# jaeyoungchoilab/Topsicle

Measured on AMD Instinct MI355X. Metric: bases_scanned_per_sec, higher is better.
Workload: dtype u8

## Files before the change

### __graft_entry__.py

```python
import os
import shutil
import subprocess
import sys

ROOT = os.path.dirname(os.path.abspath(__file__))
CSRC = os.path.join(ROOT, "topsicle_amd", "csrc")
LIB = os.path.join(ROOT, "topsicle_amd", "libtopsicle_hip.so")


def _newer(target, deps):
    return os.path.exists(target) and all(os.path.getmtime(target) >= os.path.getmtime(d) for d in deps)


HIP_FLAGS = ["--offload-arch=gfx950", "-O3", "-fno-vectorize", "-std=c++17", "-fPIC", "-Wall", "-Wno-unused-variable"]
KGROUPS = 18


def _build_hip_split(out, extra=()):
    hipcc = shutil.which("hipcc") or "/opt/rocm/bin/hipcc"
    flags = os.environ.get("TPS_HIPCC_EXTRA", "").split() + HIP_FLAGS + list(extra)
    bdir = os.path.join(CSRC, "_build", os.path.splitext(os.path.basename(out))[0])
    os.makedirs(bdir, exist_ok=True)
    jobs = []
    for g in range(KGROUPS):
# ... 24 lines not shown
    out = os.path.join(ROOT, "topsicle_amd", "libtopsicle_io.so")
    if not force and _newer(out, [src, os.path.join(CSRC, "tps_pack.h"), os.path.join(CSRC, "tps_gzpar.h"), os.path.join(ROOT, "include", "topsicle_hip.h")]):
        return out
    subprocess.check_call(["g++", "-O2", "-std=c++17", "-shared", "-fPIC", "-Wall", "-o", out, src, "-lz", "-lpthread"])
    return out


def build_oracle():
    mk = os.path.join(ROOT, "oracle", "Makefile")
    if os.path.exists(mk):
        subprocess.check_call(["make", "-s", "-C", os.path.join(ROOT, "oracle")])


def build_emulation():
    sys.path.insert(0, os.path.join(ROOT, "tests"))
    sys.path.insert(0, ROOT)
    import emu_adapter_driver
    import emu_anchor_driver
    import emu_binseg_driver
    import emu_clear_driver
    import emu_driver
    import emu_ends_driver
    import emu_follow_wide_driver
    import emu_motif_driver
    import emu_place_driver
    import emu_refine_driver
    import emu_tract_driver
    import emu_variant_driver
    import emu_wide_driver
    emu_driver.build()
    emu_binseg_driver.build()
    emu_wide_driver.build()
    emu_wide_driver.build_main()
    emu_follow_wide_driver.build()
    emu_motif_driver.build()
    emu_motif_driver.build_main()
    emu_variant_driver.build()
    emu_variant_driver.build_main()
    emu_tract_driver.build()
    emu_tract_driver.build_main()
    emu_ends_driver.build()
    emu_ends_driver.build_main()
    emu_anchor_driver.build()
    emu_anchor_driver.build_main()
    emu_place_driver.build()
    emu_place_driver.build_main()
    emu_adapter_driver.build()
    emu_adapter_driver.build_main()
    emu_refine_driver.build()
    emu_refine_driver.build_main()
    emu_clear_driver.build_main()
    import test_layout
    test_layout.build_main()

# ... 111 lines not shown
```

### topsicle_amd/csrc/topsicle_hip.hip

```cpp
#include <hip/hip_runtime.h>
#include <hip/hip_ext.h>

#include <sys/uio.h>
#include <unistd.h>

#include <algorithm>
#include <cerrno>
#include <cstdarg>
#include <cstdio>
#include <cstdlib>
#include <cstring>
#include <deque>
#include <initializer_list>
#include <map>
#include <mutex>
#include <set>
#include <string>
#include <vector>

#include "tps_device.h"
#include "tps_motif.h"
#include "tps_variant.h"
#include "tps_tract.h"
#include "tps_ends.h"
// ... 371 lines not shown
    size_t table_rr = 0;
    DevBuf follow_picks, follow_hist;
    DevBuf motif_hits, motif_counts;
    DevBuf variant_in, variant_counts, variant_prof;
    std::vector<unsigned long long> h_variant_prof;
    DevBuf tract_table, tract_out;
    DevBuf ends_in, ends_out;
    DevBuf links_t, links_out;
    DevBuf window_out;
    DevBuf offsets_in, offsets_out;
    DevBuf place_in, place_idx, place_out;
    DevBuf adapter_in, adapter_out;
    DevBuf refine_in, refine_out;
    DevBuf ascii, ascii_off;
    DevBuf nib, nib_src;
    std::set<void*> pinned;
    std::vector<tps_read_desc> h_desc;
    tps::PatInfo pat{};
    bool have_pat = false;
    Slot slots[TPS_MAX_SLOTS + 1];
    std::vector<EventPair> ev_pool;
    size_t ev_used = 0;
    size_t ev_base = 0;
    tps::PlanKnobs knobs{};
    int want_stamps = 0;
    int no_events = 0;
    int no_inline_rows = 0;
    int no_stride = 0;
    int file_order = 0;
    int poison = 0;
    int event_stride = 1;
    uint64_t launch_seq = 0;
    size_t lds_set_refine = 0;
    size_t lds_set_generic = 0;
    size_t lds_set_fused[KF_COUNT][KSLIDE_MAX - KSLIDE_MIN + 1] = {};
    uint32_t* h_flag = nullptr;
    hipEvent_t share_ev = nullptr;
    void* raw_stage[2] = {nullptr, nullptr};
    hipEvent_t raw_ev[2] = {nullptr, nullptr};
};

namespace {

int bind(tps_ctx* c) {
    if (!c) return fail(TPS_E_ARG, "null context");
    HIP_TRY(hipSetDevice(c->device));
    return TPS_OK;
// ... 1585 lines not shown
    double tot = 0.0;
    for (size_t i = c->ev_base; i < c->ev_used; ++i) {
        float ms = 0.f;
        HIP_TRY(hipEventElapsedTime(&ms, c->ev_pool[i].a, c->ev_pool[i].b));
        tot += ms;
    }
    const size_t cnt = c->ev_used - c->ev_base;
    if (n_launches) *n_launches = (int32_t)cnt;
    if (total_ms) *total_ms = tot;
    if (mean_ms) *mean_ms = cnt ? tot / (double)cnt : 0.0;
    return TPS_OK;
}

int tps_ctx_debug_option(tps_ctx* c, const char* key, int64_t value) {
    if (!c || !key) return fail(TPS_E_ARG, "null argument");
    const std::string k(key);
    if (k == "event_stride") c->event_stride = (int)std::max<int64_t>(1, value);
    else if (k == "no_events") c->no_events = value != 0;
    else if (k == "force_generic") c->knobs.force_generic = value != 0;
    else if (k == "spans_per_tile") c->knobs.spans_per_tile = (int)std::max<int64_t>(0, value);
    else if (k == "force_pair") c->knobs.force_pair = value != 0;
    else if (k == "so_order") c->knobs.so_order = (int)value;
    else if (k == "wpg") c->knobs.wpg = (int)value;
    else if (k == "stamps") c->want_stamps = value != 0;
    else if (k == "file_order") c->file_order = value != 0;
    else if (k == "no_stride") c->no_stride = value != 0;
    else if (k == "no_inline_rows") c->no_inline_rows = value != 0;
    else if (k == "poison") {
        if (value < 0 || value > 255) return fail(TPS_E_ARG, "poison must be 0 (off) or a fill byte 1..255");
        c->poison = (int)value;
    }
    else return fail(TPS_E_ARG, "unknown debug option '%s' (event_stride, no_events, force_generic, spans_per_tile, force_pair, so_order, wpg, stamps, file_order, no_stride, no_inline_rows, poison)", key);
    drop_plans(c);
    return TPS_OK;
}

int tps_debug_stamps_get(tps_ctx* c, int32_t slot, uint64_t* out, int64_t n) {
    Slot* sl;
    int rc;
    if ((rc = need_scanned(c, slot, &sl))) return rc;
    if (!sl->stamps.p || n != sl->n) return fail(TPS_E_STATE, "no stamps recorded");
    HIP_TRY(hipMemcpy(out, sl->stamps.p, (size_t)n * 16 * 8, hipMemcpyDeviceToHost));
    return TPS_OK;
}

int tps_kernel_time_reset(tps_ctx* c) {
    int rc;
    if ((rc = bind(c))) return rc;
    HIP_TRY(hipStreamSynchronize(c->stream));
    c->ev_base = c->ev_used;
    c->launch_seq = 0;
    return TPS_OK;
}

}
// ... 1 lines not shown
```

### topsicle_amd/csrc/tps_device.h

```cpp
#pragma once
#include <stdint.h>
#include "../../include/topsicle_hip.h"
#include "tps_wave.h"
#include "tps_check.h"

namespace tps {

constexpr int WPG = 4;
constexpr int WPG_MAX = 8;
constexpr uint32_t FLAG_CONFLICT = 0x80000000u;
constexpr uint32_t FLAG16 = 0x8000u;
constexpr int HIST_COPIES = 8;
constexpr int WIN_U = 4;
constexpr int COOP_MAX = 24;

typedef unsigned __int128 u128;

constexpr int cgcd(int a, int b) { return b == 0 ? a : cgcd(b, a % b); }
constexpr int clog2(int x) { return x <= 1 ? 0 : 1 + clog2(x / 2); }

struct PatInfo {
    int32_t P, k;
    uint32_t kmask;
    uint32_t all_mask;
// ... 38 lines not shown
    int32_t blk_log2;
    int32_t rec_rs;
    int32_t tot_dw;
    int32_t blk_dw;
    int32_t lc_cap;
    uint32_t jump_magic;
    int32_t q, r, lw;
    int32_t lc_global;
    int32_t lc_stride;
    uint16_t* lc_scratch;
    int32_t pair_n;
    int32_t tw;
    int32_t tile_full;
    int32_t wpg;
    int32_t pp_d;
    int32_t so_fast;
    int32_t val_on;
    int32_t seq_alias;
    int32_t lut_fields;
    int32_t lut16;
    int32_t xt_alias;
    int32_t xt_own;
    int32_t pair16;
};

struct BinsegArgs {
    const int32_t* sums;
    const int64_t* win_off;
    int32_t* bkp;
    double* gain;
    int64_t n_reads;
    int32_t n_patterns, jump, min_size;
    uint8_t* tie;
};

constexpr int MISC_DW = 20;
constexpr int XS_DW = 64 + NT + 4 * NT + NT + 16 * 5 + 8;
constexpr int HIST_STRIDE = 33;
constexpr int HIST_DW = 2 * HIST_COPIES * HIST_STRIDE;
struct Lds {
    uint32_t* lut;
    uint32_t* lut2;
    int lshift;
    uint32_t* seq2;
    uint16_t* val;
    uint32_t* blk;
    uint32_t* G;
    uint32_t* Gp;
    uint16_t* C0;
    uint16_t* C1;
    uint32_t* XPC;
    uint32_t* XF;
    uint32_t* XT;
    uint32_t* Tot;
    uint32_t* row;
    uint32_t* misc;
};
constexpr int XLANES = NT + 16;
TPS_HD int64_t xchg_dw(const ScanArgs& a) {
    return 9ll * NT + (a.xt_alias == 2 ? 0ll : 2ll) * XLANES;
}
TPS_HD int64_t lut_dw(const ScanArgs& a) { return a.lut16 ? ((((int64_t)a.lut_n + 1) / 2 + 3) & ~3ll) : (((int64_t)a.lut_n + 3) & ~3ll); }
TPS_HD int64_t blk_region_dw(const ScanArgs& a) {
    int64_t need = a.variant ? xchg_dw(a) : 2ll * a.nblk_cap + 2ll * ((a.nblk_cap + 1) / 2);
    if (need < XS_DW) need = XS_DW;
    if (need < HIST_DW) need = HIST_DW;
    return (need + 3) & ~3ll;
}
TPS_HD int64_t val_dw(const ScanArgs& a) { return a.val_on ? ((a.seq_dw + 4 + 3) / 4) * 2 : 0; }
TPS_HD int64_t row_dw(const ScanArgs& a) {
    const int64_t fused = a.variant ? ((int64_t)NT << a.blk_log2) + NT : 0;
    return fused > WIN_U * NT ? fused : WIN_U * NT;
}
TPS_DEV Lds carve(uint32_t* base, uint32_t* lut, const ScanArgs& a) {
    Lds l;
    l.lut2 = lut - a.pair_n;
    uint32_t* p = base;
    l.blk = p;  p += a.blk_dw;
    l.lut = lut;
    l.lshift = a.variant ? 16 : 0;
    l.seq2 = p; p += a.seq_dw;
    l.val = (uint16_t*)p;  p += val_dw(a);
    l.Tot = p;  p += a.tot_dw;
    l.row = p;  p += row_dw(a);
    l.misc = p;
    l.G = l.blk;
    l.Gp = l.G + a.nblk_cap;
    l.C0 = (uint16_t*)(l.Gp + a.nblk_cap);
    l.C1 = l.C0 + ((a.nblk_cap + 1) / 2) * 2;
    l.XPC = l.blk;
    l.XF = l.XPC + 9 * NT;
    l.XT = l.XF + XLANES;
    return l;
}
TPS_HD int64_t lds_dwords(const ScanArgs& a) {
    return (int64_t)a.blk_dw + (a.seq_alias ? 0 : a.seq_dw) + val_dw(a) + a.tot_dw + row_dw(a) + MISC_DW +
           ((a.xt_alias && a.xt_own) ? (a.xt_alias == 2 ? 2 : 1) * XLANES : 0);
}
TPS_HD int64_t wg_lds_dwords(const ScanArgs& a) { return a.pair_n + lut_dw(a) + (int64_t)(a.wpg > 0 ? a.wpg : WPG) * ((lds_dwords(a) + 3) & ~3ll); }
constexpr int M_BEST = 0;
constexpr int M_CMASK = 2;
constexpr int M_INVALID = 4;
constexpr int M_SCAN = 10;
constexpr int M_MAXSC = 6;
constexpr int M_BESTB = 8;
constexpr int M_NTIE = 9;
constexpr int X_Q = 0;
constexpr int X_BS = 64;
// ... 758 lines not shown
    return t;
}

template <int S>
struct Geo {
    static constexpr int B = 8;
    static constexpr int LOG2B = 3;
    static constexpr int C = 8;
    static constexpr int LOG2C = 3;
    static constexpr int POS = B * S;
    static constexpr int WDW = (POS + 13 + 15) / 16;
};
constexpr int SEQ_LEAD = 4;
template <int S, bool FULL>
struct TileGeo {
    static constexpr int LANES = FULL ? NT : NT - 1;
    static constexpr int BASES = LANES * Geo<S>::POS + 13 + 15;
    static constexpr int NQ = (63 + BASES + 63) / 64;
    static constexpr int PF = (NQ + NT - 1) / NT;
    static constexpr int SEQ_TILE = SEQ_LEAD + 4 * NQ + 4;
    static constexpr int SEQ = SEQ_TILE < 144 ? 144 : SEQ_TILE;
};
constexpr bool tile_full_default(int s) { return s >= 1; }

template <int S, bool FULL>
TPS_DEV Lds carve_fused(uint32_t* base, uint32_t* lut, const ScanArgs& a) {
    constexpr int BLK = 9 * NT, ROW = NT * Geo<S>::B + NT, SEQ = TileGeo<S, FULL>::SEQ;
    const int VAL = a.val_on ? ((SEQ + 4 + 3) / 4) * 2 : 0;
    static_assert(BLK % 4 == 0 && ROW % 4 == 0 && MISC_DW % 4 == 0 && SEQ % 4 == 0, "seq2 must be 16-byte aligned");
    static_assert(BLK + ROW - SEQ >= HIST_DW && BLK + ROW - SEQ >= 4 * NT, "step 1 counts in front of the aliased bases");
    Lds l;
    l.lut2 = lut - a.pair_n;
    l.lut = lut;
    l.lshift = (a.lut16 && !a.lut_fields && !a.pair16) ? LUT_M16 : (a.lut_fields && a.lut16) ? LUT_F16 : a.lut_fields ? LUT_FIELDS : 16;
    l.blk = base;
    l.XPC = base;
    l.G = l.Gp = base; l.C0 = l.C1 = (uint16_t*)base;
    l.row = base + BLK;
    l.misc = l.row + ROW;
    l.Tot = l.misc + MISC_DW;
    uint32_t* p = l.Tot + 4;
    if (a.seq_alias) {
        l.seq2 = base + (BLK + ROW - SEQ);
    } else {
        l.seq2 = p;
        p += SEQ;
    }
    l.val = (uint16_t*)p;
    p += VAL;
    l.XF = p;
    l.XT = l.XF + XLANES;
    return l;
}

TPS_DEV uint32_t pack_hi_lo(uint32_t hi_src, uint32_t lo_src) { return perm(hi_src, lo_src, 0x07060100u); }

template <int S, bool SO, bool INV, int RPT, bool RAW>
TPS_DEV void tile_fused_s(const ScanArgs& a, const TileConst& tc, const Lds& l, int delta, int w0, int tile, int nw_tile,
                          int64_t out_base, uint64_t& s_total, int64_t r) {
    constexpr bool RZ = RPT == 0;
    typedef Geo<S> g_;
    constexpr int WDW = g_::WDW, B = g_::B, LOG2B = g_::LOG2B, POS = g_::POS;
    constexpr int RS = NT + NT / B;
    const PatInfo& pat = a.pat;
    const int rp = RPT >= 0 ? RPT : tc.r, q = tc.q;
// ... 686 lines not shown
            }
        } else {
            TPS_EMU_COUNT(6);
        }
    }
    const Lane<uint32_t> lexc = wave_excl_sum(ltot);
    bool lane_cands = false;
    if constexpr (CD == 0 && !M16) lane_cands = tc.jump >= 4u;
    const uint32_t c_lo = div_jump((uint32_t)w0 + tc.jump - 1u, tc.jump_magic);
    uint32_t c_hi = div_jump((uint32_t)(w0 + nw_tile) + tc.jump - 1u, tc.jump_magic);
    if (c_hi > tc.lc_cap) c_hi = tc.lc_cap;
    TPS_PHASE {
        const int lane = tid;
        const uint32_t* const sw = TPS_AT(sw_);
        if constexpr (SWP) g_store_sw8p(tc.sw16 + w0, lane, nw_tile, TPS_AT(swp_));
        else g_store_sw8(tc.sw16 + w0, lane, nw_tile, sw);
        uint32_t* pr = l.row + lane * (B + 1);
        uint32_t run = 0;
        TPS_UNROLL
        for (int j = 0; j < B; ++j) { pr[j] = run; run += sw[j]; }
        xt_at(lane) = TPS_AT(lexc);
        if (lane_cands) {
            if (tid == 0) TPS_EMU_COUNT(7);
            auto own_candidates = [&](auto bigj_) {
                const uint32_t carry = (uint32_t)s_total + TPS_AT(lexc);
                const uint32_t wa = (uint32_t)w0 + (uint32_t)(lane * B);
                const uint32_t c = mulhi32(wa + tc.jump - 1u, tc.jump_magic);
                const uint32_t f = c * tc.jump - wa, f2 = f + tc.jump;
                uint32_t i1 = c, r1 = f;
                if constexpr (decltype(bigj_)::value != 0) {
                    i1 = f < (uint32_t)B ? c : c_hi;
                    r1 = f < (uint32_t)B ? f : (uint32_t)(B - 1);
                }
                const uint32_t i2 = (f2 < (uint32_t)B ? c : c_hi) + 1u;
                const uint32_t r2 = f2 < (uint32_t)B ? f2 : (uint32_t)(B - 1);
                const uint32_t v1 = pr[r1], v2 = pr[r2];
                g32_store_clamped(tc.lc_g, c_hi, i1, carry + v1);
                g32_store_clamped(tc.lc_g, c_hi, i2, carry + v2);
            };
            if (tc.jump > (uint32_t)B) own_candidates(IntC<1>());
            else own_candidates(IntC<0>());
        }
    }
    TPS_SYNC();
    if (w0 == 0) TPS_STAMP(12);
    TPS_ISA_MARK(MK + 4);
    const uint32_t gsum = uniform(l.row[nw_tile + (nw_tile >> LOG2B)] + xt_at(nw_tile >> LOG2B));
    {
        const uint32_t jump = tc.jump;
        const int passes = (c_hi > c_lo && !lane_cands) ? (int)((c_hi - c_lo + NT - 1) / NT) : 0;
        TPS_ISA_MARK(MK + 6);
        TPS_PHASE {
            const uint32_t carry = (uint32_t)s_total;
            if (tid == 0) { l.misc[M_INVALID] = 0; l.misc[M_NTIE] = 0; }
            uint32_t c = c_lo + (uint32_t)tid;
            uint32_t w = c * jump - (uint32_t)w0;
            TPS_NOVEC
            for (int t = 0; t < passes; ++t) {
                if (c < c_hi) {
                    const uint32_t pre = l.row[w + (w >> LOG2B)] + xt_at((int)(w >> LOG2B));
                    g32_store(tc.lc_g, c, carry + pre);
                }
                c += NT;
                w += NT * jump;
// ... 643 lines not shown
        const int best_b = TPS_AT(best_b_);
        double m;
        __builtin_memcpy(&m, &misc[M_MAXSC], 8);
        const double thr = m * (1.0 - 1e-14);
        uint32_t near = (best >= thr && best >= 0.0 ? 1u : 0u) + (second >= thr && second >= 0.0 ? 1u : 0u);
        if (near) lds_add(&misc[M_NTIE], near);
        if (best == m && best_b >= 0) lds_max_i32((int32_t*)&misc[M_BESTB], best_b);
    }
    TPS_SYNC();
    tie = misc[M_NTIE] > 1u;
    if (tie) {
        Cand ex = binseg_exact_wg(S, n, jump, min_size, xs);
        bkp = ex.b;
        gain = ex.b < 0 ? 0.0 : gain_from((int64_t)ex.d, ex.den, n, n_patterns);
    } else {
        bkp = (int32_t)misc[M_BESTB];
        double m;
        __builtin_memcpy(&m, &misc[M_MAXSC], 8);
        gain = bkp < 0 ? 0.0 : m / (double)n / ((double)n_patterns * (double)n_patterns);
        TPS_SYNC();
    }
}

template <typename ST>
TPS_DEV void binseg_from_lc(const ScanArgs& a, const Lds& l, uint64_t lc_g, const ST* S_global, int n, uint64_t tot, int jump,
                            int min_size, int n_patterns, uint32_t* misc, uint32_t* xs, int& bkp, double& gain, bool& tie) {
    const int ncand = (n - 1) / jump;
    Lane<double> best_(-1.0);
    Lane<int> best_b_(-1);
    Lane<bool> amb_(false);
    Lane<uint64_t> bits_(0);
    const int c_min = (min_size + jump - 1) / jump > 1 ? (min_size + jump - 1) / jump : 1;
    const int c_max = (n - min_size) / jump < ncand ? (n - min_size) / jump : ncand;
    const bool exact53 = (double)n * 4294967296.0 < 9007199254740992.0 && (double)tot * (double)n < 9007199254740992.0;
    const double nf = (double)n, totf = (double)tot;
    const bool int_d = (double)tot * (double)n < 2147483648.0 && tot < (1ull << 24);
    constexpr int LCV = 16;
    const bool prefilter = exact53 && c_max - c_min < LCV * NT;
    int nslot = c_max >= c_min ? (c_max - c_min + NT) / NT : 0;
    TPS_PIN_S(nslot);
    Lane<float> p_s1_(-1.0f), p_s2_(-1.0f);
    Lane<uint32_t> p_lc_(0);
    Lane<int> p_c_(-1);
    float thr32 = -1.0f;
    bool crowded = false;
    TPS_ISA_REGION(5);
    if (prefilter) {
        auto prefilter_phase = [&](auto intd_) {
        TPS_PHASE {
            constexpr bool INTD = decltype(intd_)::value != 0;
            float &p_s1 = TPS_AT(p_s1_), &p_s2 = TPS_AT(p_s2_);
            uint32_t& p_lc = TPS_AT(p_lc_);
            p_s1 = -1.0f; p_s2 = -1.0f; p_lc = 0;
            int p_j = -1;
            const int c0 = c_min + tid;
            const uint32_t off0 = 4u * (uint32_t)c0;
            const float nf32 = (float)n, bstep = (float)(NT * jump);
            float bf = (float)(c0 * jump);
            const uint32_t ntb_step = 0u - (uint32_t)tot * (uint32_t)(NT * jump);
            uint32_t ntb = 0u - (uint32_t)tot * (uint32_t)(c0 * jump);
            auto slot = [&](int j, uint32_t lc, auto last_) {
                float d32;
                if constexpr (INTD) {
                    d32 = (float)(int32_t)(mul24((uint32_t)n, lc) + ntb);
                    ntb += ntb_step;
                } else {
                    d32 = (float)__builtin_fma(-totf, (double)bf, nf * (double)lc);
                }
                const float den32 = bf * (nf32 - bf);
                bf += bstep;
                float s_ = d32 * d32 * rcp_f32(den32);
                if constexpr (decltype(last_)::value != 0) s_ = tid <= c_max - c_min - j * NT ? s_ : -1.0f;
                const bool gt = s_ > p_s1;
                p_s2 = med3_f32(p_s1, p_s2, s_);
                p_lc = gt ? lc : p_lc;
                p_j = gt ? j : p_j;
                p_s1 = gt ? s_ : p_s1;
            };
            auto group = [&](int g, auto checked_) {
                constexpr bool CHECKED = decltype(checked_)::value != 0;
                uint32_t lcv[4];
                TPS_UNROLL
                for (int i = 0; i < 4; ++i) {
                    const uint32_t joff = 4u * NT * (uint32_t)(4 * g + i);
                    if constexpr (CHECKED) lcv[i] = g32_load_at(lc_g, off0 + joff < 4u * (uint32_t)c_max ? off0 + joff : 4u * (uint32_t)c_max);
                    else lcv[i] = g32_load_at(lc_g + joff, off0);
                }
                TPS_UNROLL
                for (int i = 0; i < 4; ++i) slot(4 * g + i, lcv[i], checked_);
            };
            if constexpr (INTD) {
                if (nslot > 4) group(0, IntC<0>()); else if (nslot > 0) group(0, IntC<1>());
                if (nslot > 8) group(1, IntC<0>()); else if (nslot > 4) group(1, IntC<1>());
                if (nslot > 12) group(2, IntC<0>()); else if (nslot > 8) group(2, IntC<1>());
                if (nslot > 12) group(3, IntC<1>());
            } else {
                if (nslot > 0) group(0, IntC<1>());
                if (nslot > 4) group(1, IntC<1>());
                if (nslot > 8) group(2, IntC<1>());
                if (nslot > 12) group(3, IntC<1>());
            }
            TPS_AT(p_c_) = p_j >= 0 ? c0 + p_j * NT : -1;
        }
        };
        if (int_d) {
            prefilter_phase(IntC<1>());
        } else {
            TPS_EMU_COUNT(11);
            prefilter_phase(IntC<0>());
        }
        float m32;
        {
            Lane<uint32_t> key;
            TPS_LANES {
                const float nn = TPS_AT(p_s1_) > 0.0f ? TPS_AT(p_s1_) : 0.0f;
                __builtin_memcpy(&TPS_AT(key), &nn, 4);
            }
            const uint32_t mb = wave_max_u32(key);
            __builtin_memcpy(&m32, &mb, 4);
        }
        thr32 = m32 * (1.0f - 1e-4f);
        Lane<bool> close2;
        TPS_LANES { TPS_AT(close2) = TPS_AT(p_s2_) >= thr32 && TPS_AT(p_s2_) >= 0.0f; }
        crowded = wave_ballot(close2) != 0;
        if (crowded) TPS_EMU_COUNT(10);
    }
    uint64_t close = 0;
    if (prefilter) {
        Lane<bool> cl;
        TPS_LANES { TPS_AT(cl) = TPS_AT(p_c_) >= 0 && TPS_AT(p_s1_) >= thr32; }
        close = wave_ballot(cl);
    }
// ... 54 lines not shown
            __builtin_memcpy(&m, &mbits, 8);
            Lane<bool> n1, n1_amb;
            TPS_LANES {
                const double best = TPS_AT(best_);
                const bool amb = TPS_AT(amb_), near = best >= m * (1.0 - 1e-14) && best >= 0.0;
                TPS_AT(n1) = near;
                TPS_AT(n1_amb) = near && amb;
            }
            ntie = (uint32_t)__builtin_popcountll(wave_ballot(n1)) + (uint32_t)__builtin_popcountll(wave_ballot(n1_amb));
            TPS_LANES {
                const double best = TPS_AT(best_);
                const int best_b = TPS_AT(best_b_);
                TPS_AT(key) = (best == m && best_b >= 0) ? (uint32_t)best_b + 1u : 0u;
            }
            bestb = (int32_t)wave_max_u32(key) - 1;
        }
    }
    (void)misc; (void)a; (void)l;
    TPS_ISA_REGION(7);
    if (crowded) ntie = 2u;
    tie = ntie > 1u;
    if (ntie > 1u) {
        TPS_EMU_COUNT(4);
        Cand ex = binseg_exact_wg(S_global, n, jump, min_size, xs);
        bkp = ex.b;
        gain = ex.b < 0 ? 0.0 : gain_from((int64_t)ex.d, ex.den, n, n_patterns);
    } else {
        bkp = bestb;
        gain = bkp < 0 ? 0.0 : m / (double)n / ((double)n_patterns * (double)n_patterns);
    }
}

template <int SV, bool SO, bool PAIR = false, bool RAW = true, bool FULL = tile_full_default(SV), int DCLASS = 0>
TPS_DEV void scan_read(const ScanArgs& a, int64_t r, uint32_t* lds_base, uint32_t* lut) {
    constexpr bool M16K = SV != 0 && SO && !RAW;
    constexpr bool F16K = SV != 0 && SO && RAW && DCLASS == 3;
    constexpr bool P16K = SV != 0 && !SO && !RAW && PAIR && DCLASS == 4;
    Lds l_ = SV ? carve_fused<SV ? SV : 5, FULL>(lds_base, lut, a) : carve(lds_base, lut, a);
    if constexpr (P16K) l_.lshift = LUT_M16;
    const Lds l = l_;
    const PatInfo& pat = a.pat;
    const tps_params& prm = a.prm;
    const int64_t woff = a.desc[r].word_off;
    const int64_t L = a.desc[r].len;
    const bool has_inv = (a.desc[r].flags & TPS_RD_HAS_INVALID) != 0;
    const bool step1 = (prm.flags & TPS_F_STEP1) != 0;

    const int n1 = (int)(L < prm.no_bp ? L : prm.no_bp);
    const Stage st_s = stage_plan(a.seq2, a.inv, woff, L, false, 0, 0, n1);
    const Stage st_e = stage_plan(a.seq2, a.inv, woff, L, true, 0, 0, n1);

    TPS_STAMP(0);
    TPS_PHASE { for (int i = tid; i < MISC_DW; i += NT) l.misc[i] = 0; }
    TPS_SYNC();
    TPS_STAMP(1);
    TPS_PHASE {
        if (step1) {
            const int hq = a.head_dw >> 2;
            const int side = tid >> 5;
            const Stage& st = side ? st_e : st_s;
            uint32_t* dst = l.seq2 + side * a.head_dw;
// ... 306 lines not shown
                    if (tc.r == 0) tile_fused_s<SF, SO, false, 0, RAW>(a, tc, l, fdelta, w0, tile, nw_tile, out_base, s_total, r);
                    else tile_fused_s<SF, SO, false, -1, RAW>(a, tc, l, fdelta, w0, tile, nw_tile, out_base, s_total, r);
                } else {
#define TPS_TILE_RP(N) case N: if constexpr (N < SF) { if ((tc.q & 7) == 0) tile_lc_s<SF, false, (N < SF ? N : 0), PAIR, true, 0, P16K>(a, tc, l, fdelta, w0, tile, nw_tile, out_base, s_total, r); \
                                                       else tile_lc_s<SF, false, (N < SF ? N : 0), PAIR, false, 0, P16K>(a, tc, l, fdelta, w0, tile, nw_tile, out_base, s_total, r); } break;
                    switch (tc.r) {
                        TPS_TILE_RP(0) TPS_TILE_RP(1) TPS_TILE_RP(2) TPS_TILE_RP(3) TPS_TILE_RP(4) TPS_TILE_RP(5) TPS_TILE_RP(6) TPS_TILE_RP(7)
                        TPS_TILE_RP(8) TPS_TILE_RP(9) TPS_TILE_RP(10) TPS_TILE_RP(11)
                        default: break;
                    }
#undef TPS_TILE_RP
                }
                if (w0 == 0) TPS_STAMP(8);
            }
        }
    }
    res.n_win = n_win;
    TPS_STAMP(9);

    if (n_win > 0 && (prm.flags & TPS_F_BINSEG) && binseg_admissible(n_win, prm.jump, prm.min_size)) {
        int bkp;
        double gain;
        bool tie = false;
        TPS_FENCE_WG();
        const uint64_t lc_g = a.lc_global ? (uint64_t)(uintptr_t)(a.lc_scratch + r * (int64_t)a.lc_stride) : 0ull;
        if constexpr (SV != 0)
            binseg_from_lc(a, l, lc_g, (const uint16_t*)(a.sums16 + (a.win_off16 ? a.win_off16[r] : 0)), n_win, s_total, prm.jump, prm.min_size, pat.P,
                           l.misc, l.blk, bkp, gain, tie);
        else
            binseg_from_lc(a, l, lc_g, (const int32_t*)(a.sums + (a.win_off ? a.win_off[r] : 0)), n_win, s_total, prm.jump, prm.min_size, pat.P,
                           l.misc, l.blk, bkp, gain, tie);
        res.bkp = bkp;
        res.gain = gain;
        res.flags = tie ? TPS_RES_TIE : 0u;
    }
    TPS_PHASE { if (tid == 0) a.results[r] = res; }
    TPS_STAMP(10);
}

constexpr int BINSEG_SMEM_DW = ((XS_DW + 2 + MISC_DW + NT + 3) / 4) * 4;
TPS_DEV void binseg_read(const BinsegArgs& a, int64_t r, uint32_t* smem) {
    const int64_t lo = a.win_off[r];
    const int n = (int)(a.win_off[r + 1] - lo);
    const int32_t* S = a.sums + lo;
    uint32_t* xs = smem;
    uint32_t* misc = smem + ((XS_DW + 1) / 2) * 2;
    uint32_t* bs = misc + MISC_DW;
    int bkp = -1;
    double gain = 0.0;
    bool tie = false;
// ... 193 lines not shown
```

### topsicle_amd/csrc/tps_plan.h

```cpp
#pragma once
#include <cstdlib>
#include <algorithm>
#include <cstdint>
#include <cstring>
#include <string>
#include <vector>

#include "tps_device.h"

namespace tps {

inline int64_t window_count(int64_t L, int W, int s, int t, int M) {
    int64_t m = std::min<int64_t>(L, M);
    int64_t ns = m - t;
    if (W < 1 || s < 1 || ns < W) return 0;
    return (ns - W) / s + 1;
}

inline void plan_dispatch_order(const int64_t* n_win, const uint8_t* passes, int64_t n, std::vector<int32_t>& order) {
    order.clear();
    if (n < 2 || n > 0x7FFFFFFFll) return;
    constexpr int NCLS = 64;
    int64_t mx = 0;
    for (int64_t i = 0; i < n; ++i) if (passes[i] && n_win[i] > mx) mx = n_win[i];
// ... 134 lines not shown
            if (ok) mul = m;
        }
        if (!mul) return "no collision-free hash for this pattern table";
        lut.assign((size_t)2 * H, 0u);
        for (uint32_t i = 0; i < H; ++i) lut[2 * i] = 0xFFFFFFFFu;
        for (int p = 0; p < P; ++p) {
            const uint32_t slot = (codes[(size_t)p] * mul) >> (32 - log2h);
            lut[2 * slot] = codes[(size_t)p];
            lut[2 * slot + 1] = code_mask[(size_t)p];
        }
        pi.hash_mul = mul;
        pi.hash_shift = 32 - log2h;
    }
    for (int d = 1; d < k; ++d)
        if (per_pat[d]) {
            if (pi.n_periods == 8) return "pattern table has more than 8 distinct self-overlap periods";
            pi.period[pi.n_periods] = d;
            pi.period_pat[pi.n_periods] = per_pat[d];
            ++pi.n_periods;
        }
    return "";
}

inline int fused_seq_dw(int slide) {
    const int bases = NT * 8 * slide + 13 + 15;
    const int nq = (63 + bases + 63) / 64;
    const int seq = SEQ_LEAD + 4 * nq + 4;
    return seq < 144 ? 144 : seq;
}

inline void plan_wpg(ScanArgs& a, int64_t budget_dw, int max_waves_simd = 8) {
    auto waves_per_cu = [&](int w) {
        a.wpg = w;
        const int64_t dw = wg_lds_dwords(a);
        if (dw > budget_dw) return 0;
        const int64_t gran = std::max<int64_t>(1, (dw * 4 + 1279) / 1280);
        const int64_t wgs = std::min<int64_t>(std::min<int64_t>(8, 128 / gran), (4 * max_waves_simd) / w);
        return (int)std::min<int64_t>(32, wgs * w);
    };
    int best = WPG, best_w = waves_per_cu(WPG);
    if (lut_dw(a) * 4 >= 8192 || (a.pair16 && (a.pair_n + lut_dw(a)) * 4 >= 8192)) {
        const int v = waves_per_cu(WPG_MAX);
        if (v > best_w) { best = WPG_MAX; best_w = v; }
    }
    a.wpg = best;
}


inline bool has_specialised_slide(int s) { return s == 5 || s == 6 || s == 7 || s == 8; }
inline bool has_default_only_slide(int s) { return s == 3 || s == 4 || (s >= 9 && s <= 12); }

struct PlanKnobs {
    int spans_per_tile = 0;
    int force_generic = 0;
    int force_pair = 0;
    int so_order = 0;
    int wpg = 0;
};

inline std::string plan_geometry_core(ScanArgs& a, const tps_params& prm, int k, int P, int64_t max_nwin, int64_t budget_dw, const PlanKnobs& kn);
inline std::string plan_geometry(ScanArgs& a, const tps_params& prm, int k, int P, int64_t max_nwin, int64_t budget_dw,
                                 const PlanKnobs& kn = PlanKnobs()) {
    a.wpg = WPG;
    std::string err = plan_geometry_core(a, prm, k, P, max_nwin, budget_dw, kn);
    if (err.empty() && a.variant && !a.pat.hash_shift) {
        const int64_t single_bytes = (int64_t)a.lut_n * (a.lut16 ? 2 : 4);
        if ((single_bytes & (single_bytes - 1)) != 0 || ((int64_t)a.pair_n * 4) % single_bytes != 0)
            err = "LDS plan: the single table (" + std::to_string(single_bytes) + " B) would not be aligned behind a pair table of " + std::to_string((int64_t)a.pair_n * 4) + " B";
    }
    if (err.empty()) {
        const bool raw = (prm.flags & TPS_F_STORE_RAW) != 0;
        plan_wpg(a, budget_dw, !a.variant ? 8 : raw ? 5 : a.pat.so_mask != 0 ? 6 : 8);
        if ((kn.wpg == WPG || kn.wpg == WPG_MAX) && a.variant) {
            const int32_t keep = a.wpg;
            a.wpg = kn.wpg;
            if (wg_lds_dwords(a) > budget_dw) a.wpg = keep;
        }
    }
    return err;
}
inline std::string plan_geometry_core(ScanArgs& a, const tps_params& prm, int k, int P, int64_t max_nwin, int64_t budget_dw, const PlanKnobs& kn) {
// ... 9 lines not shown
        const int64_t occ_max = a.lw > 0 ? (a.lw - 1) / min_per + 1 : 0;
        if ((prm.flags & TPS_F_STORE_RAW) && occ_max > 255)
            return "raw counts are bytes: a pattern can occur " + std::to_string(occ_max) + " times in a window of " +
                   std::to_string(prm.window) + " (max 255); use a smaller --windowSize with --rawcountpattern";
        const int64_t sw_max = (int64_t)P * ((a.lw + k - 1) / k + 1);
        if (max_nwin * sw_max >= (1ll << 32)) return "window sums of one read exceed 32 bits (windows per read x window size too large)";
        if ((double)max_nwin * (double)max_nwin * (double)max_nwin * (double)sw_max >= 147573952589676412928.0 )
            return "change-point arithmetic would exceed 128 bits (windows per read x window size too large)";
    }
    const int jump = std::max(prm.jump, 1);
    a.lc_cap = (int)(max_nwin / jump + 2);
    a.jump_magic = jump == 1 ? 0u : (uint32_t)(((1ull << 32) + (uint64_t)jump - 1) / (uint64_t)jump);
    a.head_dw = 4 * ((prm.no_bp + 63 + 63) / 64) + 4;
    int max_period = 0;
    for (int i = 0; i < a.pat.n_periods; ++i) max_period = std::max(max_period, a.pat.period[i]);
    const bool sw16_ok = (int64_t)P * ((a.lw + k - 1) / k + 1) < 65536;
    const int one_period = (a.pat.dup_mask == 0 && k >= 4 && a.pat.n_periods == 1 && a.pat.period[0] >= 2 && 2 * a.pat.period[0] >= k) ? a.pat.period[0] : 0;
    const bool p16_ok = P == 16 && a.pat.dup_mask == 0 && !(prm.flags & TPS_F_STORE_RAW) &&
                        (a.pat.so_mask == 0 || (!a.val_on && one_period > 0 && one_period <= prm.slide && a.lw <= 255));
    const bool fused = !force_generic && spans_pref <= 0 && k <= TPS_DIRECT_K && (has_specialised_slide(prm.slide) || (has_default_only_slide(prm.slide) && a.pat.so_mask == 0 && !(prm.flags & TPS_F_STORE_RAW))) &&
                       (P <= 15 || p16_ok) && a.q >= 8 && sw16_ok &&
                       a.q / 8 + 2 < (XLANES - NT) && max_period <= std::min(prm.slide, 6) &&
                       2 * a.head_dw <= fused_seq_dw(prm.slide);
    a.tw = 0; a.pair_n = 0; a.lc_global = 0; a.lc_stride = 0; a.pp_d = -1; a.so_fast = 0; a.seq_alias = 0; a.lut_fields = 0; a.tile_full = 0;
    a.lut16 = 0; a.xt_alias = 0; a.xt_own = 0; a.pair16 = 0;
    if (fused) {
        const bool pp_counts = a.pat.dup_mask == 0 && k >= 4 && P <= 14 && (8 * prm.slide + k - 1) / k <= 14 && (prm.slide + k - 1) / k <= 2 &&
                               a.lw / k + 2 <= 127;
        if (pp_counts && a.pat.n_periods == 0) a.pp_d = 0;
        if (pp_counts && a.pat.n_periods == 1 && a.pat.period[0] >= 2 && 2 * a.pat.period[0] >= k) a.pp_d = a.pat.period[0];
        if (!(prm.flags & TPS_F_STORE_RAW) && P > 14 && one_period > 0) a.pp_d = one_period;
        a.lut_fields = (a.pp_d >= 0 && (prm.flags & TPS_F_STORE_RAW)) ? 1 : 0;
        a.so_fast = kn.so_order == 2 ? 2 : 1;
        if (!(prm.flags & TPS_F_STORE_RAW) && a.pp_d > 0 && a.lw > 255) a.so_fast = 0;
        if (a.pat.so_mask != 0 && !(prm.flags & TPS_F_STORE_RAW)) {
            a.lut16 = 1;
            a.xt_alias = 2;
            a.xt_own = (a.val_on || !a.so_fast || a.pp_d <= 0) ? 1 : 0;
        }
        if (prm.flags & TPS_F_STORE_RAW) {
            if (a.lut_fields && a.pat.so_mask != 0 && a.pp_d > 0 && a.lut_n >= 4096) a.lut16 = 1;
            a.xt_alias = 2;
            a.xt_own = (a.val_on || (a.pat.so_mask != 0 ? a.pp_d <= 0 : a.pp_d != 0)) ? 1 : 0;
        }
        if (a.pat.so_mask == 0 && !(prm.flags & TPS_F_STORE_RAW)) { a.xt_alias = 2; a.xt_own = 0; }
        a.variant = prm.slide;
        a.blk_log2 = 3;
// ... 16 lines not shown
        a.pair16 = 0;
        if (a.pat.so_mask == 0 && a.pat.dup_mask == 0 && k == 5 && P <= 15 && has_specialised_slide(prm.slide) && !(prm.flags & TPS_F_STORE_RAW)) {
            a.pair16 = 1;
            a.lut16 = 1;
            a.pair_n = (1 << (2 * (k + 1))) / 2;
        }
        a.blk_dw = (int32_t)blk_region_dw(a);
        if (a.pair_n && !kn.force_pair) {
            auto waves_per_cu = [&](int w) {
                const int32_t w0 = a.wpg;
                a.wpg = w;
                const int64_t dw = wg_lds_dwords(a);
                a.wpg = w0;
                if (dw > budget_dw) return 0;
                return (int)(std::min<int64_t>(8, 128 / std::max<int64_t>(1, (dw * 4 + 1279) / 1280)) * w);
            };
            const int with_pair = a.pair16 ? std::max(waves_per_cu(WPG), waves_per_cu(WPG_MAX)) : waves_per_cu(WPG);
            const int32_t keep = a.pair_n;
            const int32_t keep16 = a.pair16;
            a.pair_n = 0;
            if (keep16) { a.lut16 = 0; a.pair16 = 0; }
            if (with_pair >= 5 * WPG || waves_per_cu(WPG) <= with_pair) { a.pair_n = keep; if (keep16) { a.pair16 = 1; a.lut16 = 1; } }
        }
        if (wg_lds_dwords(a) <= budget_dw) return "";
        a.tw = 0; a.pair_n = 0; a.lc_global = 0; a.lc_stride = 0; a.pp_d = -1; a.so_fast = 0; a.seq_alias = 0; a.lut_fields = 0;
        a.lut16 = 0; a.xt_alias = 0; a.xt_own = 0; a.pair16 = 0;
    }
    a.variant = 0;
    a.lc_global = 1;
    a.lc_stride = 2 * ((a.lc_cap + 1) & ~1);
    const int g = gcd_i(prm.slide, 16);
    a.span_dw = prm.slide / g;
    const int bps = 16 / g;
    a.blk_log2 = 0;
    while ((1 << a.blk_log2) < bps) ++a.blk_log2;
    const int max_spans = 2 * NT;
    const int min_spans = (a.q + 2 + bps - 1) / bps;
    const int64_t need_blk = max_nwin + a.q + 1;
    const int need_spans = (int)std::min<int64_t>((need_blk + bps - 1) / bps, max_spans);
    int spans = spans_pref > 0 ? std::min(spans_pref, max_spans) : std::min(std::max(need_spans, 1), (int)NT);
    spans = std::max(min_spans, std::min(spans, std::max(need_spans, 1)));
    if (spans > max_spans) return "window/slide combination needs " + std::to_string(spans) + " spans per tile (max " + std::to_string(max_spans) + ")";
    auto fill = [&](int sp) {
        a.spans_per_tile = sp;
        a.nblk_cap = sp * bps;
        a.rec_rs = 0;
        a.tot_dw = std::max(((sp + 2) / 2) * 2, (int)NT);
        a.seq_dw = (std::max(sp * a.span_dw + 8, 2 * a.head_dw) + 3) & ~3;
// ... 36 lines not shown
```

### topsicle_amd/csrc/tps_wave.h

```cpp
#pragma once
#include <stdint.h>

#ifdef TPS_EMU
#define TPS_DEV static inline
#define TPS_HD static inline
#define TPS_AT(x) ((x).v[tid])
#define TPS_PHASE for (int tid = 0; tid < tps::NT; ++tid)
#define TPS_LANES for (int tid = 0; tid < tps::NT; ++tid)
#define TPS_PHASE_WITH(ln) for (int tid = (ln) * 0; tid < tps::NT; ++tid)
#define TPS_SYNC() ((void)0)
#define TPS_FENCE_WG() ((void)0)
#define TPS_UNROLL
#define TPS_NOVEC
#define TPS_PIN_S(x) ((void)0)
#define TPS_PIN_V(x) ((void)0)
#else
#define TPS_DEV __device__ __forceinline__
#define TPS_HD __host__ __device__ inline
#define TPS_AT(x) (x)
__device__ __forceinline__ int tps_fresh_lane() {
    int t = (int)(threadIdx.x & 63u);
    asm volatile("" : "+v"(t));
    return t;
}
// ... 325 lines not shown
TPS_DEV uint32_t maj3(uint32_t a, uint32_t b, uint32_t c) { return __builtin_amdgcn_bitop3_b32(a, b, c, 0xE8); }
TPS_DEV uint32_t or_and(uint32_t a, uint32_t b, uint32_t c) { return __builtin_amdgcn_bitop3_b32(a, b, c, 0xA8); }
#endif

#ifdef TPS_EMU
TPS_DEV uint32_t pk_u16_sub(uint32_t a, uint32_t b) { return ((a - b) & 0xFFFFu) | (((a >> 16) - (b >> 16)) << 16); }
TPS_DEV uint32_t pk_u16_add(uint32_t a, uint32_t b) { return ((a + b) & 0xFFFFu) | (((a >> 16) + b) << 16); }
#else
typedef unsigned short tps_u16x2 __attribute__((ext_vector_type(2)));
TPS_DEV tps_u16x2 as_u16x2(uint32_t v) { return __builtin_bit_cast(tps_u16x2, v); }
TPS_DEV uint32_t pk_u16_sub(uint32_t a, uint32_t b) { return __builtin_bit_cast(uint32_t, as_u16x2(a) - as_u16x2(b)); }
TPS_DEV uint32_t pk_u16_add(uint32_t a, uint32_t b) { return __builtin_bit_cast(uint32_t, as_u16x2(a) + (tps_u16x2)((unsigned short)b)); }
#endif

#ifdef TPS_EMU
TPS_DEV u32x4 lds_load16(const uint32_t* p) { u32x4 v; v.x = p[0]; v.y = p[1]; v.z = p[2]; v.w = p[3]; return v; }
TPS_DEV void lds_store16(uint32_t* p, const u32x4& v) { p[0] = v.x; p[1] = v.y; p[2] = v.z; p[3] = v.w; }
TPS_DEV void lds_store8(uint32_t* p, const u32x2& v) { p[0] = v.x; p[1] = v.y; }
#else
TPS_DEV u32x4 lds_load16(const uint32_t* p) { return *(const u32x4*)p; }
TPS_DEV void lds_store16(uint32_t* p, const u32x4& v) { *(u32x4*)p = v; }
TPS_DEV void lds_store8(uint32_t* p, const u32x2& v) { *(u32x2*)p = v; }
#endif

constexpr int STORE_AUX = 2;
#ifdef TPS_EMU
TPS_DEV void g_store_sw8(uint16_t* tile_out, int lane, int nw_tile, const uint32_t* v) {
    for (int i = 0; i < 8; ++i)
        if (8 * lane + i < nw_tile) tile_out[8 * lane + i] = (uint16_t)v[i];
}
TPS_DEV void g_store_sw8p(uint16_t* tile_out, int lane, int nw_tile, const uint32_t* p) {
    for (int i = 0; i < 8; ++i)
        if (8 * lane + i < nw_tile) tile_out[8 * lane + i] = (uint16_t)(p[i >> 1] >> (16 * (i & 1)));
}
#else
TPS_DEV void g_store_sw8(uint16_t* tile_out, int lane, int nw_tile, const uint32_t* v) {
    typedef unsigned int v4u __attribute__((ext_vector_type(4)));
    const __amdgpu_buffer_rsrc_t rs = __builtin_amdgcn_make_buffer_rsrc((void*)tile_out, 0, ((nw_tile + 1) & ~1) * 2, 0x00020000);
    v4u t;
    t.x = v[0] | (v[1] << 16); t.y = v[2] | (v[3] << 16); t.z = v[4] | (v[5] << 16); t.w = v[6] | (v[7] << 16);
    __builtin_amdgcn_raw_buffer_store_b128(t, rs, lane * 16, 0, STORE_AUX);
}
TPS_DEV void g_store_sw8p(uint16_t* tile_out, int lane, int nw_tile, const uint32_t* p) {
    typedef unsigned int v4u __attribute__((ext_vector_type(4)));
    const __amdgpu_buffer_rsrc_t rs = __builtin_amdgcn_make_buffer_rsrc((void*)tile_out, 0, ((nw_tile + 1) & ~1) * 2, 0x00020000);
    v4u t;
// ... 32 lines not shown
```

Before: 4043 billion.

## Keep binseg candidate sums in LDS instead of global scratch for fused scans

Adds an lc_lds mode, on by default, in which the per-candidate cumulative sums written during the fused scan are stored as 16-bit values in LDS. The LDS carve reuses the region behind the staged bases, and the binseg prefilter then reads those values from LDS instead of the global lc scratch buffer. This removes global-memory round trips and one workgroup fence on the common path, at the cost of extra LDS-layout constraints and planner eligibility checks (no second-order mask, no raw stores, no pair16, jump>=4, and a bound on the sum range so 16-bit values do not wrap). An exact-tie fallback adds a fence because the scratch region is now shared.

```diff
diff --git a/__graft_entry__.py b/__graft_entry__.py
--- a/__graft_entry__.py
+++ b/__graft_entry__.py
@@ -70,6 +70,7 @@
     import emu_driver
     import emu_ends_driver
     import emu_follow_wide_driver
+    import emu_lc_lds_driver
     import emu_motif_driver
     import emu_place_driver
     import emu_refine_driver
@@ -78,6 +79,7 @@
     import emu_wide_driver
     emu_driver.build()
     emu_binseg_driver.build()
+    emu_lc_lds_driver.build()
     emu_wide_driver.build()
     emu_wide_driver.build_main()
     emu_follow_wide_driver.build()
diff --git a/topsicle_amd/csrc/topsicle_hip.hip b/topsicle_amd/csrc/topsicle_hip.hip
--- a/topsicle_amd/csrc/topsicle_hip.hip
+++ b/topsicle_amd/csrc/topsicle_hip.hip
@@ -417,7 +417,7 @@
     std::vector<EventPair> ev_pool;
     size_t ev_used = 0;
     size_t ev_base = 0;
-    tps::PlanKnobs knobs{};
+    tps::PlanKnobs knobs = tps::product_knobs();
     int want_stamps = 0;
     int no_events = 0;
     int no_inline_rows = 0;
@@ -2049,6 +2049,7 @@
     else if (k == "force_pair") c->knobs.force_pair = value != 0;
     else if (k == "so_order") c->knobs.so_order = (int)value;
     else if (k == "wpg") c->knobs.wpg = (int)value;
+    else if (k == "lc_lds") c->knobs.lc_lds = value != 0;
     else if (k == "stamps") c->want_stamps = value != 0;
     else if (k == "file_order") c->file_order = value != 0;
     else if (k == "no_stride") c->no_stride = value != 0;
@@ -2057,7 +2058,7 @@
         if (value < 0 || value > 255) return fail(TPS_E_ARG, "poison must be 0 (off) or a fill byte 1..255");
         c->poison = (int)value;
     }
-    else return fail(TPS_E_ARG, "unknown debug option '%s' (event_stride, no_events, force_generic, spans_per_tile, force_pair, so_order, wpg, stamps, file_order, no_stride, no_inline_rows, poison)", key);
+    else return fail(TPS_E_ARG, "unknown debug option '%s' (event_stride, no_events, force_generic, spans_per_tile, force_pair, so_order, wpg, lc_lds, stamps, file_order, no_stride, no_inline_rows, poison)", key);
     drop_plans(c);
     return TPS_OK;
 }
diff --git a/topsicle_amd/csrc/tps_device.h b/topsicle_amd/csrc/tps_device.h
--- a/topsicle_amd/csrc/tps_device.h
+++ b/topsicle_amd/csrc/tps_device.h
@@ -84,6 +84,7 @@
     int32_t xt_alias;
     int32_t xt_own;
     int32_t pair16;
+    int32_t lc_lds;
 };
 
 struct BinsegArgs {
@@ -117,6 +118,7 @@
     uint32_t* Tot;
     uint32_t* row;
     uint32_t* misc;
+    uint16_t* lcl;
 };
 constexpr int XLANES = NT + 16;
 TPS_HD int64_t xchg_dw(const ScanArgs& a) {
@@ -146,6 +148,7 @@
     l.Tot = p;  p += a.tot_dw;
     l.row = p;  p += row_dw(a);
     l.misc = p;
+    l.lcl = nullptr;
     l.G = l.blk;
     l.Gp = l.G + a.nblk_cap;
     l.C0 = (uint16_t*)(l.Gp + a.nblk_cap);
@@ -950,8 +953,9 @@
     static constexpr int SEQ = SEQ_TILE < 144 ? 144 : SEQ_TILE;
 };
 constexpr bool tile_full_default(int s) { return s >= 1; }
-
-template <int S, bool FULL>
+constexpr int lc_lds_entries(int seq_dw) { return 2 * (9 * NT - seq_dw); }
+
+template <int S, bool FULL, bool LCF = false>
 TPS_DEV Lds carve_fused(uint32_t* base, uint32_t* lut, const ScanArgs& a) {
     constexpr int BLK = 9 * NT, ROW = NT * Geo<S>::B + NT, SEQ = TileGeo<S, FULL>::SEQ;
     const int VAL = a.val_on ? ((SEQ + 4 + 3) / 4) * 2 : 0;
@@ -968,7 +972,20 @@
     l.misc = l.row + ROW;
     l.Tot = l.misc + MISC_DW;
     uint32_t* p = l.Tot + 4;
-    if (a.seq_alias) {
+    l.lcl = nullptr;
+    bool lc_lds = false;
+    if constexpr (LCF) lc_lds = a.lc_lds != 0;
+    if (lc_lds) {
+        static_assert(ROW == BLK, "row[] takes XPC's words");
+        static_assert(HIST_DW <= BLK && OCC_BASE_DW + 2 * OCC_SLOTS * 32 <= BLK && XS_DW <= BLK && 4 * NT <= BLK,
+                      "step 1's histograms and occurrence slots and the exact tournament's scratch in front of the staged bases");
+        static_assert(SEQ < ROW, "room for the candidate sums behind the staged bases");
+        static_assert(lc_lds_entries(SEQ) == 2 * (ROW - SEQ) && lc_lds_entries(SEQ) <= 16 * NT,
+                      "the entries the plan admits are the room the carve has; never more candidates than the prefilter takes (16 slots per lane)");
+        l.row = base;
+        l.seq2 = base + BLK;
+        l.lcl = (uint16_t*)(base + BLK + SEQ);
+    } else if (a.seq_alias) {
         l.seq2 = base + (BLK + ROW - SEQ);
     } else {
         l.seq2 = p;
@@ -1701,11 +1718,13 @@
         xt_at(lane) = TPS_AT(lexc);
         if (lane_cands) {
             if (tid == 0) TPS_EMU_COUNT(7);
-            auto own_candidates = [&](auto bigj_) {
+            auto own_candidates = [&](auto bigj_, auto lds_) {
+                constexpr bool LCL = decltype(lds_)::value != 0;
                 const uint32_t carry = (uint32_t)s_total + TPS_AT(lexc);
                 const uint32_t wa = (uint32_t)w0 + (uint32_t)(lane * B);
-                const uint32_t c = mulhi32(wa + tc.jump - 1u, tc.jump_magic);
+                uint32_t c = mulhi32(wa + tc.jump - 1u, tc.jump_magic);
                 const uint32_t f = c * tc.jump - wa, f2 = f + tc.jump;
+                if constexpr (LCL) c = c < c_hi ? c : c_hi;
                 uint32_t i1 = c, r1 = f;
                 if constexpr (decltype(bigj_)::value != 0) {
                     i1 = f < (uint32_t)B ? c : c_hi;
@@ -1714,11 +1733,20 @@
                 const uint32_t i2 = (f2 < (uint32_t)B ? c : c_hi) + 1u;
                 const uint32_t r2 = f2 < (uint32_t)B ? f2 : (uint32_t)(B - 1);
                 const uint32_t v1 = pr[r1], v2 = pr[r2];
-                g32_store_clamped(tc.lc_g, c_hi, i1, carry + v1);
-                g32_store_clamped(tc.lc_g, c_hi, i2, carry + v2);
+                if constexpr (LCL) {
+                    if (tid == 0) TPS_EMU_COUNT(15);
+                    lds16_store(l.lcl, i1, carry + v1);
+                    lds16_store(l.lcl, i2, carry + v2);
+                } else {
+                    g32_store_clamped(tc.lc_g, c_hi, i1, carry + v1);
+                    g32_store_clamped(tc.lc_g, c_hi, i2, carry + v2);
+                }
             };
-            if (tc.jump > (uint32_t)B) own_candidates(IntC<1>());
-            else own_candidates(IntC<0>());
+            if (a.lc_lds) {
+                if (tc.jump > (uint32_t)B) own_candidates(IntC<1>(), IntC<1>());
+                else own_candidates(IntC<0>(), IntC<1>());
+            } else if (tc.jump > (uint32_t)B) own_candidates(IntC<1>(), IntC<0>());
+            else own_candidates(IntC<0>(), IntC<0>());
         }
     }
     TPS_SYNC();
@@ -2408,9 +2436,11 @@
     }
 }
 
-template <typename ST>
+template <typename ST, bool LCL = false>
 TPS_DEV void binseg_from_lc(const ScanArgs& a, const Lds& l, uint64_t lc_g, const ST* S_global, int n, uint64_t tot, int jump,
                             int min_size, int n_patterns, uint32_t* misc, uint32_t* xs, int& bkp, double& gain, bool& tie) {
+    bool lc_lds = false;
+    if constexpr (LCL) lc_lds = a.lc_lds != 0;
     const int ncand = (n - 1) / jump;
     Lane<double> best_(-1.0);
     Lane<int> best_b_(-1);
@@ -2432,9 +2462,11 @@
     bool crowded = false;
     TPS_ISA_REGION(5);
     if (prefilter) {
-        auto prefilter_phase = [&](auto intd_) {
+        auto prefilter_phase = [&](auto intd_, auto lds_) {
         TPS_PHASE {
             constexpr bool INTD = decltype(intd_)::value != 0;
+            constexpr bool LDSC = decltype(lds_)::value != 0;
+            uint32_t lcp = 0;
             float &p_s1 = TPS_AT(p_s1_), &p_s2 = TPS_AT(p_s2_);
             uint32_t& p_lc = TPS_AT(p_lc_);
             p_s1 = -1.0f; p_s2 = -1.0f; p_lc = 0;
@@ -2466,6 +2498,20 @@
             auto group = [&](int g, auto checked_) {
                 constexpr bool CHECKED = decltype(checked_)::value != 0;
                 uint32_t lcv[4];
+                if constexpr (LDSC) {
+                    TPS_UNROLL
+                    for (int i = 0; i < 4; ++i) {
+                        const uint32_t ci = (uint32_t)c0 + NT * (uint32_t)(4 * g + i);
+                        if constexpr (CHECKED) lcv[i] = lds16_load(l.lcl, ci < (uint32_t)c_max ? ci : (uint32_t)c_max);
+                        else lcv[i] = lds16_load(l.lcl + NT * (4 * g + i), (uint32_t)c0);
+                    }
+                    TPS_UNROLL
+                    for (int i = 0; i < 4; ++i) {
+                        lcp += (lcv[i] - lcp) & 0xFFFFu;
+                        slot(4 * g + i, lcp, checked_);
+                    }
+                    return;
+                }
                 TPS_UNROLL
                 for (int i = 0; i < 4; ++i) {
                     const uint32_t joff = 4u * NT * (uint32_t)(4 * g + i);
@@ -2489,11 +2535,16 @@
             TPS_AT(p_c_) = p_j >= 0 ? c0 + p_j * NT : -1;
         }
         };
-        if (int_d) {
-            prefilter_phase(IntC<1>());
+        if (!int_d) TPS_EMU_COUNT(11);
+        if (lc_lds) {
+            if constexpr (LCL) {
+                if (int_d) prefilter_phase(IntC<1>(), IntC<1>());
+                else prefilter_phase(IntC<0>(), IntC<1>());
+            }
+        } else if (int_d) {
+            prefilter_phase(IntC<1>(), IntC<0>());
         } else {
-            TPS_EMU_COUNT(11);
-            prefilter_phase(IntC<0>());
+            prefilter_phase(IntC<0>(), IntC<0>());
         }
         float m32;
         {
@@ -2594,6 +2645,7 @@
     tie = ntie > 1u;
     if (ntie > 1u) {
         TPS_EMU_COUNT(4);
+        if (lc_lds) TPS_FENCE_WG();
         Cand ex = binseg_exact_wg(S_global, n, jump, min_size, xs);
         bkp = ex.b;
         gain = ex.b < 0 ? 0.0 : gain_from((int64_t)ex.d, ex.den, n, n_patterns);
@@ -2608,7 +2660,8 @@
     constexpr bool M16K = SV != 0 && SO && !RAW;
     constexpr bool F16K = SV != 0 && SO && RAW && DCLASS == 3;
     constexpr bool P16K = SV != 0 && !SO && !RAW && PAIR && DCLASS == 4;
-    Lds l_ = SV ? carve_fused<SV ? SV : 5, FULL>(lds_base, lut, a) : carve(lds_base, lut, a);
+    constexpr bool LCF = SV != 0 && !SO && !RAW && !P16K;
+    Lds l_ = SV ? carve_fused<SV ? SV : 5, FULL, LCF>(lds_base, lut, a) : carve(lds_base, lut, a);
     if constexpr (P16K) l_.lshift = LUT_M16;
     const Lds l = l_;
     const PatInfo& pat = a.pat;
@@ -2961,10 +3014,12 @@
         int bkp;
         double gain;
         bool tie = false;
-        TPS_FENCE_WG();
+        bool lc_lds = false;
+        if constexpr (LCF) lc_lds = a.lc_lds != 0;
+        if (!lc_lds) TPS_FENCE_WG();
         const uint64_t lc_g = a.lc_global ? (uint64_t)(uintptr_t)(a.lc_scratch + r * (int64_t)a.lc_stride) : 0ull;
         if constexpr (SV != 0)
-            binseg_from_lc(a, l, lc_g, (const uint16_t*)(a.sums16 + (a.win_off16 ? a.win_off16[r] : 0)), n_win, s_total, prm.jump, prm.min_size, pat.P,
+            binseg_from_lc<uint16_t, LCF>(a, l, lc_g, (const uint16_t*)(a.sums16 + (a.win_off16 ? a.win_off16[r] : 0)), n_win, s_total, prm.jump, prm.min_size, pat.P,
                            l.misc, l.blk, bkp, gain, tie);
         else
             binseg_from_lc(a, l, lc_g, (const int32_t*)(a.sums + (a.win_off ? a.win_off[r] : 0)), n_win, s_total, prm.jump, prm.min_size, pat.P,
diff --git a/topsicle_amd/csrc/tps_plan.h b/topsicle_amd/csrc/tps_plan.h
--- a/topsicle_amd/csrc/tps_plan.h
+++ b/topsicle_amd/csrc/tps_plan.h
@@ -180,7 +180,7 @@
     return "";
 }
 
-inline int fused_seq_dw(int slide) {
+constexpr int fused_seq_dw(int slide) {
     const int bases = NT * 8 * slide + 13 + 15;
     const int nq = (63 + bases + 63) / 64;
     const int seq = SEQ_LEAD + 4 * nq + 4;
@@ -214,7 +214,17 @@
     int force_pair = 0;
     int so_order = 0;
     int wpg = 0;
+    int lc_lds = 0;
 };
+inline PlanKnobs product_knobs() {
+    PlanKnobs kn;
+    kn.lc_lds = 1;
+    return kn;
+}
+template <int S> constexpr bool fused_seq_dw_is_tilegeo() { return fused_seq_dw(S) == TileGeo<S, true>::SEQ; }
+static_assert(fused_seq_dw_is_tilegeo<3>() && fused_seq_dw_is_tilegeo<4>() && fused_seq_dw_is_tilegeo<5>() && fused_seq_dw_is_tilegeo<6>() &&
+              fused_seq_dw_is_tilegeo<7>() && fused_seq_dw_is_tilegeo<8>() && fused_seq_dw_is_tilegeo<9>() && fused_seq_dw_is_tilegeo<10>() &&
+              fused_seq_dw_is_tilegeo<11>() && fused_seq_dw_is_tilegeo<12>(), "fused_seq_dw(slide) == TileGeo<slide, true>::SEQ for every fused slide");
 
 inline std::string plan_geometry_core(ScanArgs& a, const tps_params& prm, int k, int P, int64_t max_nwin, int64_t budget_dw, const PlanKnobs& kn);
 inline std::string plan_geometry(ScanArgs& a, const tps_params& prm, int k, int P, int64_t max_nwin, int64_t budget_dw,
@@ -270,7 +280,7 @@
                        (P <= 15 || p16_ok) && a.q >= 8 && sw16_ok &&
                        a.q / 8 + 2 < (XLANES - NT) && max_period <= std::min(prm.slide, 6) &&
                        2 * a.head_dw <= fused_seq_dw(prm.slide);
-    a.tw = 0; a.pair_n = 0; a.lc_global = 0; a.lc_stride = 0; a.pp_d = -1; a.so_fast = 0; a.seq_alias = 0; a.lut_fields = 0; a.tile_full = 0;
+    a.tw = 0; a.pair_n = 0; a.lc_global = 0; a.lc_lds = 0; a.lc_stride = 0; a.pp_d = -1; a.so_fast = 0; a.seq_alias = 0; a.lut_fields = 0; a.tile_full = 0;
     a.lut16 = 0; a.xt_alias = 0; a.xt_own = 0; a.pair16 = 0;
     if (fused) {
         const bool pp_counts = a.pat.dup_mask == 0 && k >= 4 && P <= 14 && (8 * prm.slide + k - 1) / k <= 14 && (prm.slide + k - 1) / k <= 2 &&
@@ -333,8 +343,16 @@
             if (keep16) { a.lut16 = 0; a.pair16 = 0; }
             if (with_pair >= 5 * WPG || waves_per_cu(WPG) <= with_pair) { a.pair_n = keep; if (keep16) { a.pair16 = 1; a.lut16 = 1; } }
         }
+        if (kn.lc_lds && a.pat.so_mask == 0 && !(prm.flags & TPS_F_STORE_RAW) && !a.pair16 && jump >= 4 && a.pat.dup_mask == 0) {
+            const int64_t c_min = std::max<int64_t>(((int64_t)std::max(prm.min_size, 1) + jump - 1) / jump, 1);
+            if ((int64_t)a.lc_cap + 2 <= lc_lds_entries(fused_seq_dw(prm.slide)) && (c_min + 64) * (int64_t)jump * ((int64_t)a.lw + P) < 65536) {
+                a.lc_lds = 1;
+                a.lc_global = 0;
+                a.lc_stride = 0;
+            }
+        }
         if (wg_lds_dwords(a) <= budget_dw) return "";
-        a.tw = 0; a.pair_n = 0; a.lc_global = 0; a.lc_stride = 0; a.pp_d = -1; a.so_fast = 0; a.seq_alias = 0; a.lut_fields = 0;
+        a.tw = 0; a.pair_n = 0; a.lc_global = 0; a.lc_lds = 0; a.lc_stride = 0; a.pp_d = -1; a.so_fast = 0; a.seq_alias = 0; a.lut_fields = 0;
         a.lut16 = 0; a.xt_alias = 0; a.xt_own = 0; a.pair16 = 0;
     }
     a.variant = 0;
diff --git a/topsicle_amd/csrc/tps_wave.h b/topsicle_amd/csrc/tps_wave.h
--- a/topsicle_amd/csrc/tps_wave.h
+++ b/topsicle_amd/csrc/tps_wave.h
@@ -371,6 +371,8 @@
 TPS_DEV void lds_store16(uint32_t* p, const u32x4& v) { *(u32x4*)p = v; }
 TPS_DEV void lds_store8(uint32_t* p, const u32x2& v) { *(u32x2*)p = v; }
 #endif
+TPS_DEV void lds16_store(uint16_t* base, uint32_t i, uint32_t v) { base[i] = (uint16_t)v; }
+TPS_DEV uint32_t lds16_load(const uint16_t* base, uint32_t i) { return base[i]; }
 
 constexpr int STORE_AUX = 2;
 #ifdef TPS_EMU
```

New measurement: 4412 billion, median of 6. +9.1%, better.
